# NikolausDemmel/rootba

Hardware: NVIDIA H100
Metric: ms/LM-iter (linearize+QR+PCG) on BAL at 1/2/4/8 H100 vs CPU ref (lower is better)
Workload: dtype f32

## Files before the change

### rootba_b200/csrc/assembled.cuh

```cuda
#pragma once

#include "kernels.cuh"

namespace rba {

template <class S>
__global__ void __launch_bounds__(256) k_rcs_terms(const S* __restrict__ panel, const AsmTerm* __restrict__ terms, long long nt,
                                                   int damping, S* __restrict__ stage, const int* __restrict__ done) {
  using V2 = typename ST<S>::V2;
  if (*done) return;
  const int lane = threadIdx.x & 31;
  const int g = lane / 9, p = lane - 9 * g;
  if (lane >= 27) return;
  const long long warps = (long long)gridDim.x * (blockDim.x >> 5);
  for (long long w = 3 * (blockIdx.x * (long long)(blockDim.x >> 5) + (threadIdx.x >> 5)) + g; w < nt; w += 3 * warps) {
    const AsmTerm at = terms[w];
    const int n = at.meta & 0x7fff, lg = (at.meta >> 15) & 7, KP = at.meta >> 18, G = 1 << lg;
    const int ia = at.ij & 0xffff, ib = at.ij >> 16;
    const int ca = 9 * ia + p, pa = ca >> 1;
    const int off_a = 2 * ((pa >> lg) * 32 + (pa & (G - 1))) + (ca & 1);
    const int cb0 = 9 * ib, pb0 = cb0 >> 1;
    const bool odd = cb0 & 1;
    int off_b[5];
#pragma unroll
// ... 19 lines not shown
    S* o = stage + 81 * (size_t)w + 9 * p;
#pragma unroll
    for (int q = 0; q < 9; ++q) o[q] = acc[q];
  }
}

template <class S>
__global__ void k_rcs_combine(const int* __restrict__ blk_ptr, const int* __restrict__ wpos, int nblk, const S* __restrict__ stage,
                              S* __restrict__ out, const int* __restrict__ done) {
  if (*done) return;
  const long long i = blockIdx.x * (long long)blockDim.x + threadIdx.x;
  if (i >= 81LL * nblk) return;
  const int bi = (int)(i / 81), e = (int)(i - 81LL * bi);
  const S* st = stage + e;
  S s = 0;
  for (int t = blk_ptr[bi]; t < blk_ptr[bi + 1]; ++t) s += st[81 * (size_t)wpos[t]];
  out[i] = s;
}

constexpr int DMP_WARPS = 4;
constexpr int DMP_BATCH = 16;
template <class S>
__global__ void __launch_bounds__(DMP_WARPS * 32) k_rcs_damping(const int* __restrict__ blk_ptr, const int2* __restrict__ terms, int nblk,
                                                                 const S* __restrict__ dmp, const S* __restrict__ base,
                                                                 const int2* __restrict__ pos, S* __restrict__ out,
                                                                 const int* __restrict__ done) {
  constexpr int B = DMP_BATCH, NV = 28 * sizeof(S) / 16;
  constexpr int ROUNDS = (2 * B * NV + 31) / 32;
  __shared__ __align__(16) S rec[DMP_WARPS][B][2][28];
  if (*done) return;
  const int w = threadIdx.x >> 5, lane = threadIdx.x & 31;
  const int bi = blockIdx.x * DMP_WARPS + w;
  if (bi >= nblk) return;
  const bool own = lane < 27;
  const int p = lane / 3, q = 3 * (lane - 3 * p);
  S s[3] = {0, 0, 0};
  if (own) {
#pragma unroll
    for (int u = 0; u < 3; ++u) s[u] = base[81 * (size_t)bi + 3 * lane + u];
  }
  int4* rv = reinterpret_cast<int4*>(&rec[w][0][0][0]);
  const int t1 = blk_ptr[bi + 1];
  for (int t0 = blk_ptr[bi]; t0 < t1; t0 += B) {
    const int nb = min(B, t1 - t0);
    int4 v[ROUNDS];
#pragma unroll
    for (int c = 0; c < ROUNDS; ++c) {
      const int i = lane + 32 * c, r = i / NV, k = i - r * NV;
      v[c] = make_int4(0, 0, 0, 0);
      if (i < 2 * nb * NV) {
        const int2 tt = __ldg(terms + t0 + (r >> 1));
        v[c] = __ldg(reinterpret_cast<const int4*>(dmp + 28 * (size_t)(r & 1 ? tt.y : tt.x)) + k);
      }
    }
#pragma unroll
    for (int c = 0; c < ROUNDS; ++c)
      if (lane + 32 * c < 2 * nb * NV) rv[lane + 32 * c] = v[c];
    __syncwarp();
    if (own) {
      for (int j = 0; j < nb; ++j) {
        const S* a = rec[w][j][0];
        const S* b = rec[w][j][1];
#pragma unroll
        for (int u = 0; u < 3; ++u) {
          S t = fma(a[p], b[q + u], S(0));
          t = fma(a[9 + p], b[9 + q + u], t);
          t = fma(a[18 + p], b[18 + q + u], t);
          s[u] += t;
        }
      }
    }
    __syncwarp();
  }
  if (own) {
    S* o = out + 81 * (size_t)pos[bi].x + 3 * lane;
#pragma unroll
    for (int u = 0; u < 3; ++u) o[u] = s[u];
  }
}

template <class S>
__global__ void k_rcs_mirror(const int2* __restrict__ pos, int nblk, S* val, const int* __restrict__ done) {
  if (*done) return;
  const long long i = blockIdx.x * (long long)blockDim.x + threadIdx.x;
  if (i >= 81LL * nblk) return;
  const int bi = (int)(i / 81), e = (int)(i - 81LL * bi);
  const int2 ps = pos[bi];
  if (ps.y >= 0) val[81 * (size_t)ps.y + e] = val[81 * (size_t)ps.x + 9 * (e % 9) + e / 9];
}

constexpr int SPMV_WARPS = 4;
constexpr int SPMV_UNROLL = 4;
template <class S>
__global__ void __launch_bounds__(SPMV_WARPS * 32) k_rcs_spmv(const int* __restrict__ row_ptr, const int* __restrict__ col,
                                                               const S* __restrict__ val, const S* __restrict__ x, S* __restrict__ y,
                                                               const int* done, int pdl) {
  __shared__ S part[SPMV_WARPS][81];
  if (done && *reinterpret_cast<const volatile int*>(done)) return;
  const int row = blockIdx.x, w = threadIdx.x >> 5, lane = threadIdx.x & 31;
  const int k0 = row_ptr[row], k1 = row_ptr[row + 1];
  int qe[3];
#pragma unroll
  for (int u = 0; u < 3; ++u) qe[u] = (lane + 32 * u) % 9;
  if (pdl) asm volatile("griddepcontrol.wait;" ::: "memory");
  if (done && *done) return;
  if (pdl) asm volatile("griddepcontrol.launch_dependents;" ::: "memory");
  S acc[3] = {0, 0, 0};
  for (int k = k0 + w; k < k1; k += SPMV_WARPS * SPMV_UNROLL) {
    S v[SPMV_UNROLL][3], xv[SPMV_UNROLL][3];
#pragma unroll
    for (int j = 0; j < SPMV_UNROLL; ++j) {
      const int kk = k + SPMV_WARPS * j;
      const bool in = kk < k1;
      const S* blk = val + 81 * (size_t)(in ? kk : k0);
      const S* xc = x + 9 * (size_t)(in ? __ldg(col + kk) : 0);
#pragma unroll
      for (int u = 0; u < 3; ++u) {
        const bool e_in = in && lane + 32 * u < 81;
        v[j][u] = e_in ? __ldg(blk + lane + 32 * u) : S(0);
        xv[j][u] = e_in ? __ldcg(xc + qe[u]) : S(0);
      }
    }
#pragma unroll
    for (int j = 0; j < SPMV_UNROLL; ++j)
#pragma unroll
      for (int u = 0; u < 3; ++u) acc[u] = fma(v[j][u], xv[j][u], acc[u]);
  }
#pragma unroll
  for (int u = 0; u < 3; ++u)
    if (lane + 32 * u < 81) part[w][lane + 32 * u] = acc[u];
  __syncthreads();
  if (threadIdx.x < 9) {
    const int p = threadIdx.x;
    S s = 0;
#pragma unroll
    for (int ww = 0; ww < SPMV_WARPS; ++ww)
#pragma unroll
      for (int q = 0; q < 9; ++q) s += part[ww][9 * p + q];
    y[9 * (size_t)row + p] = s;
  }
}

}
```

### rootba_b200/csrc/solver.cu

```cuda
#include <cuda_runtime.h>
#include <dlfcn.h>

#include <cstdio>
#include <cstdlib>
#include <cstring>
#include <chrono>
#include <array>
#include <limits>
#include <memory>
#include <string>
#include <vector>

#include "../../include/rootba_b200.h"
#include "../host/bal_io_fast.hpp"
#include "kernels.cuh"
#include "covariance.cuh"
#include "assembled.cuh"
#include "groups.cuh"
#include "nccl_dyn.hpp"

namespace rba {

thread_local std::string g_err;

// ... 152 lines not shown
  S* d_pair_ov = nullptr;
  int n_lmp = 0, lmp_cap = 0;
  int* d_lmp_slot = nullptr;
  int* d_lmp_of_lm = nullptr;
  int* d_lmp_lm = nullptr;
  S* d_lmp_mean = nullptr;
  S* d_lmp_L = nullptr;
  S* d_lmp_Lg = nullptr;
  int n_groups = 0;
  std::vector<int> h_grp_lead;
  std::vector<uint8_t> h_fixed;
  int* d_grp_lead = nullptr; int* d_grp_ptr = nullptr; int* d_grp_mem = nullptr;
  uint8_t* d_grp_fixed = nullptr;
  S* d_grp_ve = nullptr;
  S* d_grp_y = nullptr;
  S* d_obs_W = nullptr;
  rba_stage_timings tm{};
  EventPair ev_stage1, ev_stage2, ev_precond, ev_pcg, ev_backsub, ev_update, ev_error, ev_mv, ev_user;
  long long launches = 0;
  long long lin_l0 = 0, solve_l0 = 0, apply_l0 = 0;
  NcclApi* nccl = nullptr;
  ncclComm_t comm = nullptr;
  char* peer_mem = nullptr;
  size_t peer_bytes = 0;
  PeerComm pc{};
  bool peer_ok = false;
  int ar_seq = 0, c_seq = 0, s_seq = 0;
  std::vector<void*> ipc_opened;
  bool cov_ready = false;
  int cov_nblk = 0;
  IntPair* d_cov_blk_cam = nullptr; int* d_cov_blk_ptr = nullptr; IntPair* d_cov_terms = nullptr;
  int* d_cov_lm_slot0 = nullptr; int* d_cov_lm_n = nullptr;
  bool asm_on = false, su_valid = false, s_valid = false, su_new = false;
  int asm_nblk = 0, asm_switch = 0; long long asm_nt = 0, asm_nnzb = 0;
  AsmTerm* d_asm_terms = nullptr; int* d_asm_wpos = nullptr; int* d_asm_blk_ptr = nullptr; IntPair* d_asm_pos = nullptr;
  IntPair* d_asm_slots = nullptr;
  int* d_asm_row_ptr = nullptr; int* d_asm_col = nullptr;
  S* d_asm_stage = nullptr; S* d_asm_Su = nullptr; S* d_asm_S = nullptr;

  ~Solver() override {
    if (comm && nccl) nccl->CommDestroy(comm);
    for (void* p : ipc_opened) cudaIpcCloseMemHandle(p);
    for (void* p : allocs) cudaFree(p);
    if (h_prog) cudaFreeHost(h_prog);
    if (h_state) cudaFreeHost(h_state);
    if (h_res) cudaFreeHost(h_res);
    for (EventPair* e : {&ev_stage1, &ev_stage2, &ev_precond, &ev_pcg, &ev_backsub, &ev_update, &ev_error, &ev_mv, &ev_user}) {
      if (e->a) cudaEventDestroy(e->a);
      if (e->b) cudaEventDestroy(e->b);
    }
    for (auto& e : poll_ev) if (e) cudaEventDestroy(e);
    if (stream) cudaStreamDestroy(stream);
  }

  template <class T>
  int dalloc(T** p, size_t count, bool zero = true) {
    const size_t bytes = std::max<size_t>(count, 1) * sizeof(T);
    void* q = nullptr;
    CU(cudaMalloc(&q, bytes));
    allocs.push_back(q);
    device_bytes += bytes;
    if (zero) CU(cudaMemsetAsync(q, 0, bytes, stream));
    *p = (T*)q;
    return RBA_OK;
  }
  int dfree(void* q) {
    if (!q) return RBA_OK;
    allocs.erase(std::find(allocs.begin(), allocs.end(), q));
    CU(cudaFree(q));
    return RBA_OK;
  }
// ... 38 lines not shown
    TRY(alloc_buffers());
    TRY(setup_assembled());
    TRY(setup_kernels());
    CU(cudaStreamSynchronize(stream));
    return RBA_OK;
  }

  int validate_options(const rba_solver_opts& o) {
    opt = o;
    if (opt.nranks < 1 || opt.rank < 0 || opt.rank >= opt.nranks) { g_err = "bad rank/nranks"; return RBA_ERR_INVALID_ARGUMENT; }
    if (opt.operator_form != 0 && opt.operator_form != 1) { g_err = "operator_form must be 0 (dense) or 1 (implicit)"; return RBA_ERR_INVALID_ARGUMENT; }
    if (opt.solver_type < 0 || opt.solver_type > 2) { g_err = "solver_type must be 0 (SQUARE_ROOT), 1 (SCHUR_COMPLEMENT) or 2 (POWER_SCHUR_COMPLEMENT)"; return RBA_ERR_INVALID_ARGUMENT; }
    if (opt.solver_type == 2 && opt.nranks > 1) { g_err = "POWER_SCHUR_COMPLEMENT runs on one GPU (the power-series vector kernel has no peer exchange yet)"; return RBA_ERR_UNSUPPORTED; }
    if (opt.stage2_form != 0 && opt.stage2_form != 1) { g_err = "stage2_form must be 0 (Q2 panel, reference) or 1 (orthogonality identity)"; return RBA_ERR_INVALID_ARGUMENT; }
    if (opt.pcg_check_period <= 0) opt.pcg_check_period = 4;
    if (opt.residual_reset_period <= 0) opt.residual_reset_period = 10;
    if (opt.power_order <= 0) opt.power_order = 20;
    panels = opt.operator_form == 0 && opt.solver_type == 0;
    ko.use_valid_projections_only = opt.use_valid_projections_only;
    ko.robust_norm = opt.robust_norm;
    ko.write_panel = panels;
    ko.huber = opt.huber_parameter;
    ko.jacobi_eps = opt.jacobi_scaling_epsilon > 0 ? opt.jacobi_scaling_epsilon : (double)ST<S>::eps_sqrt();
    return RBA_OK;
  }
  bool panel_form() const { return panels && opt.stage2_form == 0; }

  void read_test_hooks() {
    if (const char* e = getenv("RBA_PCG_PARTIALS")) pcg_partials = atoi(e) != 0;
    if (const char* e = getenv("RBA_PCG_CLUSTER")) pcg_cluster = std::max(1, std::min(atoi(e), 16));
    if (const char* e = getenv("RBA_PEER_AR")) peer_ar = atoi(e) != 0;
    if (const char* e = getenv("RBA_ASSEMBLED_RCS")) asm_hook = atoi(e) != 0;
    if (const char* e = getenv("RBA_ASSEMBLED_AT")) asm_at = std::max(0, atoi(e));
  }

  int upload_layout(const rba_problem_view* pv) {
    nc = pv->num_cameras;
    nl_total = pv->num_landmarks;
    nobs_total = pv->lm_obs_offset[nl_total];
    std::string msg = build_layout(nc, nl_total, pv->lm_obs_offset, pv->obs_cam_idx, opt.rank, opt.nranks, KPMAX, L);
    if (!msg.empty()) { g_err = msg; return RBA_ERR_INVALID_ARGUMENT; }
    std::vector<S> xy((size_t)2 * L.nslots, S(0));
    const S* src = (const S*)pv->obs_xy;
    for (int s = 0; s < L.nslots; ++s)
      if (L.slot_obs[s] >= 0) { xy[2 * (size_t)s] = src[2 * L.slot_obs[s]]; xy[2 * (size_t)s + 1] = src[2 * L.slot_obs[s] + 1]; }
    TileInfo* d_tiles; int* d_sorted; int* d_slot_cam; int* d_slot_lm; S* d_xy;
    TRY(upload(&d_tiles, L.tiles));
    TRY(upload(&d_sorted, L.sorted_lm));
    TRY(upload(&d_slot_cam, L.slot_cam));
    TRY(upload(&d_slot_lm, L.slot_lm));
    TRY(upload(&d_xy, xy));
    D.tiles = d_tiles; D.ntiles = (int)L.tiles.size(); D.sorted_lm = d_sorted;
    D.slot_cam = d_slot_cam; D.slot_lm = d_slot_lm; D.slot_xy = d_xy; D.nslots = L.nslots; D.nc = nc;
    TRY(upload(&d_csr_obs_slots, L.csr_obs.slots));
    TRY(upload(&d_csr_obs_items, L.csr_obs.items));
    TRY(upload(&d_csr_obs_item_ptr, L.csr_obs.cam_item_ptr));
    n_obs_items = (int)L.csr_obs.items.size();
    if (L.csr_y_is_obs) {
      d_csr_y_slots = d_csr_obs_slots; d_csr_y_items = d_csr_obs_items; d_csr_y_item_ptr = d_csr_obs_item_ptr;
      n_y_items = n_obs_items;
    } else {
      TRY(upload(&d_csr_y_slots, L.csr_y.slots));
      TRY(upload(&d_csr_y_items, L.csr_y.items));
      TRY(upload(&d_csr_y_item_ptr, L.csr_y.cam_item_ptr));
      n_y_items = (int)L.csr_y.items.size();
    }
// ... 762 lines not shown
  }

  int precond_blocks(int mode, S* dst, const S* addend, bool reduce_ranks) {
    const int g = (n_pb_items + 127) / 128;
    switch (mode) {
      case 0: k_precond_partial<S, 0><<<g, 128, 0, stream>>>(D.jp, (const S*)nullptr, d_csr_obs_slots, d_pb_items, n_pb_items, D.pblk); break;
      case 1: k_precond_partial<S, 1><<<g, 128, 0, stream>>>(D.jp, D.q1d, d_csr_obs_slots, d_pb_items, n_pb_items, D.pblk); break;
      case 2: k_precond_partial<S, 2><<<g, 128, 0, stream>>>(D.dmp, (const S*)nullptr, d_csr_obs_slots, d_pb_items, n_pb_items, D.pblk); break;
      default: k_precond_partial<S, 3><<<g, 128, 0, stream>>>(D.blk0, (const S*)nullptr, d_csr_obs_slots, d_pb_items, n_pb_items, D.pblk); break;
    }
    k_precond_final<S><<<(45 * nc + 255) / 256, 256, 0, stream>>>(D.pblk, d_pb_item_ptr, nc, addend, dst);
    launches += 2;
    return reduce_ranks ? allreduce(dst, (size_t)81 * nc) : RBA_OK;
  }

  enum class Handover {
    Assembled,
    Partials,
    Counter,
    Peer,
    Nccl,
  };
  Handover handover() const {
    if (s_valid) return Handover::Assembled;
    if (n_groups) return opt.nranks > 1 ? Handover::Nccl : Handover::Counter;
    if (opt.nranks > 1) return peer_ok ? Handover::Peer : Handover::Nccl;
    const bool vec_cached = 9 * ((nc + pcg_cluster - 1) / pcg_cluster) <= VEC_THREADS * VEC_EPT;
    return pcg_partials && vec_cached && opt.solver_type != 2 ? Handover::Partials : Handover::Counter;
  }
  int apply_operator(const S* xvec, Handover h, bool in_solve, int e0_only = 0) {
    const int* done = in_solve ? &d_state->done : nullptr;
    const bool pdl = in_solve;
    ++tm.matvec_launches;
    if (h == Handover::Assembled)
      return launch_ex(k_rcs_spmv<S>, nc, SPMV_WARPS * 32, 0, pdl, 1, (const int*)d_asm_row_ptr, (const int*)d_asm_col, (const S*)d_asm_S, xvec, D.y, done, (int)pdl);
    if (panels) {
      if (L.n_items_large > 0) {
        k_matvec_large<S, K4_WARPS, KPMAX><<<grid_for(L.n_items_large, K4_WARPS, 4), K4_WARPS * 32, k4_smem_small, stream>>>(
            D, d_items, 0, L.n_items_large, L.k4_scratch_per_warp, xvec, done);
        ++launches;
      }
      const bool p = pdl && L.n_items_large == 0;
      if (n_dealt > L.n_items_large)
        TRY(launch_ex(k_matvec_small_tma<S, K4_WARPS, K4_NS, K4_STAGE>, tma_grid, K4_WARPS * 32, K4_SMEM_TMA, p, 1, D, (const MatvecItem*)d_items, L.n_items_large, n_dealt, xvec, done, (int)p));
    } else {
      const int ntl = (int)L.tiles.size();
      const bool p = pdl && imp_tile_split == ntl;
      if (imp_tile_split > 0)
        TRY(launch_ex((k_matvec_implicit_tma<S, IMP_WARPS, IMP_MAXSLOTS, IMP_NS>), imp_grid, IMP_WARPS * 32, imp_smem, p, 1, D, imp_tile_split, xvec, done, (int)p, e0_only));
      if (imp_tile_split < ntl)
        TRY(launch_ex(k_matvec_implicit<S>, (ntl - imp_tile_split + TILE_WARPS - 1) / TILE_WARPS, TILE_WARPS * 32, 0, false, 1, D, imp_tile_split, xvec, done, 0, e0_only));
    }
    const int grid = grid_for(n_op_items, 8, 8);
    if (h == Handover::Partials)
      return launch_ex(k_cam_reduce<S>, grid, 256, 0, pdl, 1, (const S*)D.yobs, op_slots, op_items, n_op_items, D.partial, done, (int)pdl);
    if (h == Handover::Peer) ++ar_seq;
    if (h == Handover::Nccl) CU(cudaMemsetAsync(D.y, 0, (size_t)9 * nc * sizeof(S), stream));
    auto kern = h == Handover::Peer ? k_cam_reduce_final<S, true> : k_cam_reduce_final<S, false>;
    TRY(launch_ex(kern, grid, 256, 0, pdl, 1, (const S*)D.yobs, op_slots, op_items, n_op_items, op_item_ptr, D.partial, d_cam_cnt, D.y, done, (int)pdl, pc, ar_seq, nc));
    return h == Handover::Nccl ? allreduce(D.y, (size_t)9 * nc) : RBA_OK;
  }
  int matvec_launch(const S* xvec, bool clear_y) {
    const Handover h = handover() == Handover::Assembled ? Handover::Assembled : Handover::Counter;
    if (clear_y && h == Handover::Counter) CU(cudaMemsetAsync(D.y, 0, (size_t)9 * nc * sizeof(S), stream));
    return apply_operator(xvec, h, false);
  }
  int pcg_vec(int i, int mode, bool pdl, int is_last, S lambda, bool fused_ar = false, bool from_partials = false) {
    PeerComm c = pc;
// ... 113 lines not shown
    Handover h = handover();
    if (h == Handover::Counter) CU(cudaMemsetAsync(D.y, 0, (size_t)9 * nc * sizeof(S), stream));
    if (power) return power_enqueue(h, inc_out);
    rc = start(ev_pcg); if (rc) return rc;
    CU(cudaMemsetAsync(d_state, 0, sizeof(PcgState), stream));
    const int max_it = std::max(opt.max_linear_solver_iterations, 1);
    const int period = opt.residual_reset_period;
    const int depth = opt.pcg_check_period;
    h_prog[0] = 0; h_prog[1] = 0;
    ar_seq = (++pcg_solve_id) * (2 * max_it + 4);
    rc = pcg_vec(0, 3, false, 0, lambda); if (rc) return rc;
    auto enqueue_iteration = [&](int i) -> int {
      const int is_last = (i == max_it) ? 1 : 0;
      if (i % period == 0) {
        TRY(pcg_step(i, 1, 0, lambda, h));
        return pcg_step(i, 2, is_last, lambda, h);
      }
      return pcg_step(i, 0, is_last, lambda, h);
    };
    if (h == Handover::Nccl) {
      TRY(enqueue_polled(max_it, depth, enqueue_iteration));
    } else {
      volatile int* prog = h_prog;
      for (int i = 1; i <= max_it; ++i) {
        unsigned spins = 0;
        while (!prog[1] && i - prog[0] > depth) {
          if ((++spins & 0xffffu) == 0 && cudaStreamQuery(stream) != cudaErrorNotReady) break;
        }
        if (prog[1] && i - prog[0] > depth) break;
        if (asm_on && i == asm_switch) {
          su_new = !su_valid;
          if (su_new) assemble(0);
          assemble(1);
          su_valid = s_valid = true;
          h = handover();
        }
        rc = enqueue_iteration(i); if (rc) return rc;
      }
    }
    if (n_groups) TRY(group_expand(D.inc, D.inc, false));
    CU(cudaMemcpyAsync(&h_state[0], d_state, sizeof(PcgState), cudaMemcpyDeviceToHost, stream));
    if (inc_out) CU(cudaMemcpyAsync(inc_out, D.inc, (size_t)9 * nc * sizeof(S), cudaMemcpyDeviceToHost, stream));
    rc = stop(ev_pcg); if (rc) return rc;
    have_inc = true;
    new_linearization_point = false;
    return RBA_OK;
  }
  int solve_finish(rba_cg_summary* cg) {
    CU(cudaGetLastError());
    tm.stage2_time = elapsed(ev_stage2);
    tm.compute_preconditioner_time = elapsed(ev_precond);
    tm.solve_reduced_system_time = elapsed(ev_pcg);
    tm.kernel_launches = launches - solve_l0;
    if (cg) {
      cg->termination_type = h_state[0].term;
      cg->num_iterations = h_state[0].iter;
      cg->reason = h_state[0].reason;
      cg->num_matvecs = h_state[0].iter + h_state[0].iter / opt.residual_reset_period;
    }
    if (s_valid && h_state[0].iter < asm_switch) {
      s_valid = false;
      if (su_new) su_valid = false;
    }
    if (h_state[0].reason == 99) {
      g_err = "PCG: a peer rank did not publish its operator output in time (peer-memory exchange timed out)";
      return RBA_ERR_NCCL;
    }
// ... 213 lines not shown
    CU(cudaGetLastError());
    return RBA_OK;
  }

  int time_matvec(int reps, double* sec) override {
    if (!linearized || !damping_valid) { g_err = "rba_time_matvec needs rba_linearize + rba_solve first"; return RBA_ERR_STATE; }
    TRY(matvec_launch(D.p, false));
    TRY(start(ev_mv));
    for (int r = 0; r < reps; ++r) TRY(matvec_launch(D.p, false));
    TRY(stop(ev_mv));
    CU(cudaStreamSynchronize(stream));
    CU(cudaGetLastError());
    *sec = elapsed(ev_mv) / std::max(reps, 1);
    tm.matvec_time = *sec;
    return RBA_OK;
  }

  int timer_start() override { return start(ev_user); }
  int timer_stop(double* sec) override {
    int rc = stop(ev_user); if (rc) return rc;
    CU(cudaStreamSynchronize(stream));
    *sec = elapsed(ev_user);
    return RBA_OK;
  }
  void* stream_ptr() override { return (void*)stream; }
  int synchronize() override { CU(cudaStreamSynchronize(stream)); return RBA_OK; }

  bool asm_candidate() const { return asm_hook && opt.nranks == 1 && panels; }
  int setup_assembled() {
    if (!asm_candidate()) return RBA_OK;
    PairList P;
    const std::string msg = build_pair_list(L, P);
    if (!msg.empty()) { g_err = msg; return RBA_ERR_UNSUPPORTED; }
    AsmPlan A;
    plan_assembled(L, P, sizeof(S), A);
    if (!A.fits) return RBA_OK;
    size_t free_b = 0, total_b = 0;
    CU(cudaMemGetInfo(&free_b, &total_b));
    if ((size_t)A.device_bytes + ((size_t)256 << 20) > free_b) return RBA_OK;
    TRY(upload(&d_asm_terms, A.terms));
    TRY(upload(&d_asm_wpos, P.wpos));
    TRY(upload(&d_asm_slots, P.terms));
    TRY(upload(&d_asm_blk_ptr, P.blk_ptr));
    TRY(upload(&d_asm_pos, A.pos));
    TRY(upload(&d_asm_row_ptr, A.row_ptr));
    TRY(upload(&d_asm_col, A.col));
    TRY(dalloc(&d_asm_stage, (size_t)A.nt * 81, false));
    TRY(dalloc(&d_asm_Su, (size_t)A.nblk * 81));
    TRY(dalloc(&d_asm_S, (size_t)A.nnzb * 81));
    asm_nt = A.nt; asm_nblk = (int)A.nblk; asm_nnzb = A.nnzb;
    asm_switch = asm_at > 0 ? asm_at : A.switch_iteration;
    asm_on = true;
    return RBA_OK;
  }
  void assemble(int damping) {
    const int* done = &d_state->done;
    const unsigned per_entry = (unsigned)((81LL * asm_nblk + 255) / 256);
    if (damping) {
      k_rcs_damping<S><<<(asm_nblk + DMP_WARPS - 1) / DMP_WARPS, DMP_WARPS * 32, 0, stream>>>(
          d_asm_blk_ptr, (const int2*)d_asm_slots, asm_nblk, D.dmp, d_asm_Su, (const int2*)d_asm_pos, d_asm_S, done);
      k_rcs_mirror<S><<<per_entry, 256, 0, stream>>>((const int2*)d_asm_pos, asm_nblk, d_asm_S, done);
    } else {
      const int grid = (int)std::max<long long>(1, std::min<long long>((asm_nt + 23) / 24, (long long)sm_count * 16));
      k_rcs_terms<S><<<grid, 256, 0, stream>>>(D.panel, d_asm_terms, asm_nt, 0, d_asm_stage, done);
      k_rcs_combine<S><<<per_entry, 256, 0, stream>>>(d_asm_blk_ptr, d_asm_wpos, asm_nblk, d_asm_stage, d_asm_Su, done);
    }
    launches += 2;
  }

  template <class T>
  int cov_upload(T** p, const std::vector<T>& v) {
    void* q = nullptr;
    CU(cudaMalloc(&q, std::max<size_t>(v.size(), 1) * sizeof(T)));
    allocs.push_back(q);
    if (!v.empty()) CU(cudaMemcpy(q, v.data(), v.size() * sizeof(T), cudaMemcpyHostToDevice));
    *p = (T*)q;
    return RBA_OK;
  }
  int cov_build_lists() {
    if (cov_ready) return RBA_OK;
    PairList P;
    const std::string msg = build_pair_list(L, P);
    if (!msg.empty()) { g_err = msg; return RBA_ERR_UNSUPPORTED; }
    TRY(cov_upload(&d_cov_blk_cam, P.blk_cam));
    TRY(cov_upload(&d_cov_blk_ptr, P.blk_ptr));
    TRY(cov_upload(&d_cov_terms, P.terms));
    TRY(cov_upload(&d_cov_lm_slot0, P.slot0));
    TRY(cov_upload(&d_cov_lm_n, P.nn));
    cov_nblk = (int)P.blk_cam.size();
    cov_ready = true;
    return RBA_OK;
  }
  template <bool TA, bool TB>
  void cov_gemm(long long M, long long N, long long K, double alpha, const double* A, long long lda, const double* B, long long ldb,
// ... 505 lines not shown
```

### rootba_b200/csrc/kernels.cuh

```cuda
#pragma once

#include <cooperative_groups.h>
#include <cuda_runtime.h>

#include <cfloat>
#include <cmath>
#include <cstdint>

#include "layout.hpp"

namespace rba {

template <class S> struct ST;
template <> struct ST<float> {
  using V2 = float2;
  using V4 = float4;
  __host__ __device__ static float eps_sqrt() { return 0.0031622776601683794f; }
  __host__ __device__ static float eps() { return 1e-5f; }
  __host__ __device__ static float tiny() { return FLT_MIN; }
};
template <> struct ST<double> {
  using V2 = double2;
  using V4 = double4;
  __host__ __device__ static double eps_sqrt() { return 1e-5; }
// ... 1572 lines not shown
      const V2 v = __ldg(prow + (size_t)(r * KP + k) * 32);
      const int c = 2 * lane + 64 * k;
      d += v.x * xs[c] + v.y * xs[c + 1];
    }
    d = warp_sum(d);
    for (int k = 0; k < KP; ++k) {
      const V2 v = __ldg(prow + (size_t)(r * KP + k) * 32);
      const int c = 2 * lane + 64 * k;
      ys[c] += d * v.x;
      ys[c + 1] += d * v.y;
    }
  }
  __syncwarp();
  for (int c = lane; c < ncols; c += 32) D.yobs[9 * (size_t)it.yslot_base + c] = ys[c];
  __syncwarp();
}

__device__ __forceinline__ uint32_t smem_u32(const void* p) { return (uint32_t)__cvta_generic_to_shared(p); }
__device__ __forceinline__ void mbar_init(uint64_t* bar, uint32_t count) {
  asm volatile("mbarrier.init.shared::cta.b64 [%0], %1;" ::"r"(smem_u32(bar)), "r"(count) : "memory");
}
__device__ __forceinline__ void mbar_fence_init() {
  asm volatile("fence.mbarrier_init.release.cluster;" ::: "memory");
  asm volatile("fence.proxy.async.shared::cta;" ::: "memory");
}
__device__ __forceinline__ void mbar_expect_tx(uint64_t* bar, uint32_t bytes) {
  asm volatile("mbarrier.arrive.expect_tx.shared::cta.b64 _, [%0], %1;" ::"r"(smem_u32(bar)), "r"(bytes) : "memory");
}
__device__ __forceinline__ uint64_t l2_evict_first_policy() {
  uint64_t pol;
  asm volatile("createpolicy.fractional.L2::evict_first.b64 %0, 1.0;" : "=l"(pol));
  return pol;
}
__device__ __forceinline__ void bulk_g2s(void* dst, const void* src, uint32_t bytes, uint64_t* bar, uint64_t policy) {
  asm volatile("cp.async.bulk.shared::cluster.global.mbarrier::complete_tx::bytes.L2::cache_hint [%0], [%1], %2, [%3], %4;" ::"r"(
                   smem_u32(dst)),
               "l"(src), "r"(bytes), "r"(smem_u32(bar)), "l"(policy)
               : "memory");
}
__device__ __forceinline__ void mbar_wait(uint64_t* bar, uint32_t parity) {
  uint32_t ok;
  const uint32_t a = smem_u32(bar);
  do {
    asm volatile("{\n .reg .pred p;\n mbarrier.try_wait.parity.shared::cta.b64 p, [%1], %2;\n selp.u32 %0, 1, 0, p;\n}"
                 : "=r"(ok)
                 : "r"(a), "r"(parity)
                 : "memory");
  } while (!ok);
}

template <class S>
struct PanelStream {
  const S* src;
  int rows_left;
  int row_scalars;
  int rows_per_stage;
  int next_item;
  unsigned issued;
  uint64_t policy;
};

template <class S, int NS, int STAGE_BYTES>
__device__ __forceinline__ bool stream_produce(PanelStream<S>& ps, const DevPtrs<S>& D, const MatvecItem* __restrict__ items,
                                               int item_end, int item_stride, unsigned char* ring, uint64_t* bars, int lane) {
  if (ps.rows_left == 0) {
    if (ps.next_item >= item_end) return false;
// ... 1291 lines not shown
```

### rootba_b200/csrc/layout.hpp

```cpp
#pragma once

#include <algorithm>
#include <cmath>
#include <cstdint>
#include <limits>
#include <numeric>
#include <string>
#include <utility>
#include <vector>

namespace rba {

struct TileInfo {
  long long panel_off;
  int slot_base;
  int lm_base;
  short n;
  short G;
  short KP;
  short nvalid;
};

struct MatvecItem {
  int tile;
// ... 294 lines not shown
  pass(tmp, idx, true);
  tmp.clear(); tmp.shrink_to_fit();
  P.terms.resize(raw.size());
  for (size_t t = 0; t < idx.size(); ++t) P.terms[t] = raw[idx[t]];
  P.wpos.swap(idx);
  for (size_t t = 0; t < P.terms.size(); ++t) {
    const IntPair cc{L.slot_cam[P.terms[t].x], L.slot_cam[P.terms[t].y]};
    if (t == 0 || cc.x != P.blk_cam.back().x || cc.y != P.blk_cam.back().y) {
      P.blk_cam.push_back(cc);
      P.blk_ptr.push_back((int)t);
    }
  }
  P.blk_ptr.push_back((int)P.terms.size());
  return "";
}

struct AsmTerm {
  long long base;
  int ij, meta;
};
inline AsmTerm pack_asm_term(long long base, int ia, int ib, int n, int G, int KP) {
  int lg = 0;
  while ((1 << lg) < G) ++lg;
  return {base, ia | ib << 16, n | lg << 15 | KP << 18};
}

constexpr long long ASM_STAGE_BYTES = (long long)2 << 30;

inline int asm_switch_iteration(long long nt, long long panel_scalars, long long s_bytes, int scalar_size) {
  const double staged = 4.0 * (double)nt * 81 * scalar_size, saved = (double)panel_scalars * scalar_size - (double)s_bytes;
  return 1 + (int)std::ceil(2.0 * staged / std::max(saved, 1.0));
}

struct AsmPlan {
  long long nt = 0, nblk = 0, nnzb = 0, s_bytes = 0, device_bytes = 0;
  bool fits = false;
  int switch_iteration = 0;
  std::vector<int> row_ptr;
  std::vector<int> col;
  std::vector<IntPair> pos;
  std::vector<AsmTerm> terms;
};

inline void plan_assembled(const Layout& L, const PairList& P, int scalar_size, AsmPlan& A) {
  A = AsmPlan();
  const int nc = L.nc;
  A.nblk = (long long)P.blk_cam.size();
  A.nt = (long long)P.terms.size();
  long long ndiag = 0;
  for (const IntPair& c : P.blk_cam) ndiag += c.x == c.y;
  A.nnzb = 2 * A.nblk - ndiag;
  A.s_bytes = A.nnzb * 81 * scalar_size;
  A.switch_iteration = asm_switch_iteration(A.nt, L.panel_scalars, A.s_bytes, scalar_size);
  A.fits = 4 * A.s_bytes <= L.panel_scalars * scalar_size && 81 * A.nt * scalar_size <= ASM_STAGE_BYTES;
  if (!A.fits) return;
  A.device_bytes = A.s_bytes + (A.nblk + A.nt) * 81 * scalar_size + A.nt * (long long)(sizeof(AsmTerm) + sizeof(int) + sizeof(IntPair)) +
                   (A.nblk + A.nnzb + nc + 2) * (long long)sizeof(int) + A.nblk * (long long)sizeof(IntPair);
  A.row_ptr.assign((size_t)nc + 1, 0);
  A.col.resize((size_t)A.nnzb);
  for (const IntPair& c : P.blk_cam) { ++A.row_ptr[c.x + 1]; if (c.x != c.y) ++A.row_ptr[c.y + 1]; }
  for (int c = 0; c < nc; ++c) A.row_ptr[c + 1] += A.row_ptr[c];
  std::vector<int> fill(A.row_ptr.begin(), A.row_ptr.end() - 1);
  A.pos.resize((size_t)A.nblk);
  for (long long b = 0; b < A.nblk; ++b) {
    const IntPair c = P.blk_cam[b];
    const int lo = fill[c.x]++;
    A.col[lo] = c.y;
    int up = -1;
    if (c.x != c.y) { up = fill[c.y]++; A.col[up] = c.x; }
    A.pos[b] = {lo, up};
  }
  A.terms.reserve((size_t)A.nt);
  for (int lm = 0; lm < L.nl_local; ++lm) {
    const int sidx = L.sorted_of_lm[lm];
    const TileInfo& T = L.tiles[L.tile_of_sorted[sidx]];
    const int g = sidx - T.lm_base;
    for (int a = 0; a < T.n; ++a)
      for (int b = 0; b <= a; ++b) A.terms.push_back(pack_asm_term(T.panel_off + 2LL * g * T.G, a, b, T.n, T.G, T.KP));
  }
}

}
```

Baseline: 6.013.

## Fuse mirror into damping kernel and add dedicated diagonal-block damping kernel

The separate mirror kernel is removed. The off-diagonal damping kernel now writes both the lower block and its transpose into the upper position directly. Diagonal blocks, which can carry many terms, are handled by a new block-per-diagonal kernel that prefetches term records into shared memory one batch ahead and uses the symmetric a^T a product. This removes a launch and a read-back pass and spreads the long diagonal sums across 81 threads instead of 27 lanes. The cost is strided transposed stores and an extra kernel with a software-pipelined loop.

New measurement: 5.982 (median of 6 runs). No clear change (-0.5%).

```diff
diff --git a/rootba_b200/csrc/assembled.cuh b/rootba_b200/csrc/assembled.cuh
--- a/rootba_b200/csrc/assembled.cuh
+++ b/rootba_b200/csrc/assembled.cuh
@@ -75,6 +75,8 @@
   const int w = threadIdx.x >> 5, lane = threadIdx.x & 31;
   const int bi = blockIdx.x * DMP_WARPS + w;
   if (bi >= nblk) return;
+  const int2 ps = __ldg(pos + bi);
+  if (ps.y < 0) return;
   const bool own = lane < 27;
   const int p = lane / 3, q = 3 * (lane - 3 * p);
   S s[3] = {0, 0, 0};
@@ -116,20 +118,65 @@
     __syncwarp();
   }
   if (own) {
-    S* o = out + 81 * (size_t)pos[bi].x + 3 * lane;
-#pragma unroll
-    for (int u = 0; u < 3; ++u) o[u] = s[u];
-  }
-}
-
-template <class S>
-__global__ void k_rcs_mirror(const int2* __restrict__ pos, int nblk, S* val, const int* __restrict__ done) {
-  if (*done) return;
-  const long long i = blockIdx.x * (long long)blockDim.x + threadIdx.x;
-  if (i >= 81LL * nblk) return;
-  const int bi = (int)(i / 81), e = (int)(i - 81LL * bi);
-  const int2 ps = pos[bi];
-  if (ps.y >= 0) val[81 * (size_t)ps.y + e] = val[81 * (size_t)ps.x + 9 * (e % 9) + e / 9];
+    S* lo = out + 81 * (size_t)ps.x + 3 * lane;
+    S* up = out + 81 * (size_t)ps.y + p;
+#pragma unroll
+    for (int u = 0; u < 3; ++u) {
+      lo[u] = s[u];
+      up[9 * (q + u)] = s[u];
+    }
+  }
+}
+
+constexpr int DIAG_THREADS = 96;
+constexpr int DIAG_BATCH = 32;
+template <class S>
+__global__ void __launch_bounds__(DIAG_THREADS) k_rcs_damping_diag(const int* __restrict__ diag, const int* __restrict__ blk_ptr,
+                                                                    const int2* __restrict__ terms, const S* __restrict__ dmp,
+                                                                    const S* __restrict__ base, const int2* __restrict__ pos,
+                                                                    S* __restrict__ out, const int* __restrict__ done) {
+  constexpr int B = DIAG_BATCH, NV = 28 * sizeof(S) / 16;
+  constexpr int ROUNDS = (B * NV + DIAG_THREADS - 1) / DIAG_THREADS;
+  __shared__ __align__(16) S rec[B][28];
+  if (*done) return;
+  const int bi = __ldg(diag + blockIdx.x), e = threadIdx.x;
+  const bool own = e < 81;
+  const int p = e / 9, q = e - 9 * p;
+  S s = own ? base[81 * (size_t)bi + e] : S(0);
+  const int t0 = __ldg(blk_ptr + bi), t1 = __ldg(blk_ptr + bi + 1);
+  int4 v[ROUNDS];
+  int4* rv = reinterpret_cast<int4*>(&rec[0][0]);
+  for (int t = t0 - B; t < t1; t += B) {
+    if (t >= t0) {
+      __syncthreads();
+#pragma unroll
+      for (int c = 0; c < ROUNDS; ++c)
+        if (e + DIAG_THREADS * c < min(B, t1 - t) * NV) rv[e + DIAG_THREADS * c] = v[c];
+      __syncthreads();
+    }
+    const int nf = min(B, t1 - t - B);
+#pragma unroll
+    for (int c = 0; c < ROUNDS; ++c) {
+      const int i = e + DIAG_THREADS * c, r = i / NV, k = i - r * NV;
+      v[c] = make_int4(0, 0, 0, 0);
+      if (i < nf * NV) {
+        const int slot = __ldg(reinterpret_cast<const int*>(terms + t + B + r));
+        v[c] = __ldg(reinterpret_cast<const int4*>(dmp + 28 * (size_t)slot) + k);
+      }
+    }
+    if (t < t0) continue;
+    const int nb = min(B, t1 - t);
+    if (own) {
+      for (int j = 0; j < nb; ++j) {
+        const S* a = rec[j];
+        S u = fma(a[p], a[q], S(0));
+        u = fma(a[9 + p], a[9 + q], u);
+        u = fma(a[18 + p], a[18 + q], u);
+        s += u;
+      }
+    }
+  }
+  if (own) out[81 * (size_t)__ldg(&pos[bi].x) + e] = s;
 }
 
 constexpr int SPMV_WARPS = 4;
diff --git a/rootba_b200/csrc/solver.cu b/rootba_b200/csrc/solver.cu
--- a/rootba_b200/csrc/solver.cu
+++ b/rootba_b200/csrc/solver.cu
@@ -208,10 +208,10 @@
   IntPair* d_cov_blk_cam = nullptr; int* d_cov_blk_ptr = nullptr; IntPair* d_cov_terms = nullptr;
   int* d_cov_lm_slot0 = nullptr; int* d_cov_lm_n = nullptr;
   bool asm_on = false, su_valid = false, s_valid = false, su_new = false;
-  int asm_nblk = 0, asm_switch = 0; long long asm_nt = 0, asm_nnzb = 0;
+  int asm_nblk = 0, asm_switch = 0, asm_ndiag = 0; long long asm_nt = 0, asm_nnzb = 0;
   AsmTerm* d_asm_terms = nullptr; int* d_asm_wpos = nullptr; int* d_asm_blk_ptr = nullptr; IntPair* d_asm_pos = nullptr;
   IntPair* d_asm_slots = nullptr;
-  int* d_asm_row_ptr = nullptr; int* d_asm_col = nullptr;
+  int* d_asm_row_ptr = nullptr; int* d_asm_col = nullptr; int* d_asm_diag = nullptr;
   S* d_asm_stage = nullptr; S* d_asm_Su = nullptr; S* d_asm_S = nullptr;
 
   ~Solver() override {
@@ -1619,10 +1619,14 @@
     TRY(upload(&d_asm_pos, A.pos));
     TRY(upload(&d_asm_row_ptr, A.row_ptr));
     TRY(upload(&d_asm_col, A.col));
+    std::vector<int> diag;
+    for (long long b = 0; b < A.nblk; ++b)
+      if (A.pos[b].y < 0) diag.push_back((int)b);
+    TRY(upload(&d_asm_diag, diag));
     TRY(dalloc(&d_asm_stage, (size_t)A.nt * 81, false));
     TRY(dalloc(&d_asm_Su, (size_t)A.nblk * 81));
     TRY(dalloc(&d_asm_S, (size_t)A.nnzb * 81));
-    asm_nt = A.nt; asm_nblk = (int)A.nblk; asm_nnzb = A.nnzb;
+    asm_nt = A.nt; asm_nblk = (int)A.nblk; asm_nnzb = A.nnzb; asm_ndiag = (int)diag.size();
     asm_switch = asm_at > 0 ? asm_at : A.switch_iteration;
     asm_on = true;
     return RBA_OK;
@@ -1633,7 +1637,8 @@
     if (damping) {
       k_rcs_damping<S><<<(asm_nblk + DMP_WARPS - 1) / DMP_WARPS, DMP_WARPS * 32, 0, stream>>>(
           d_asm_blk_ptr, (const int2*)d_asm_slots, asm_nblk, D.dmp, d_asm_Su, (const int2*)d_asm_pos, d_asm_S, done);
-      k_rcs_mirror<S><<<per_entry, 256, 0, stream>>>((const int2*)d_asm_pos, asm_nblk, d_asm_S, done);
+      k_rcs_damping_diag<S><<<asm_ndiag, DIAG_THREADS, 0, stream>>>(d_asm_diag, d_asm_blk_ptr, (const int2*)d_asm_slots, D.dmp, d_asm_Su,
+                                                                   (const int2*)d_asm_pos, d_asm_S, done);
     } else {
       const int grid = (int)std::max<long long>(1, std::min<long long>((asm_nt + 23) / 24, (long long)sm_count * 16));
       k_rcs_terms<S><<<grid, 256, 0, stream>>>(D.panel, d_asm_terms, asm_nt, 0, d_asm_stage, done);
```

## Rewrite assembled SpMV as persistent load-balanced kernel with bulk-copy pipeline

Applied to the files above, without the earlier changes.

Replaces the one-CTA-per-row block SpMV with a persistent grid sized by occupancy. Rows are dealt to CTAs with LPT balancing and split into fixed-size chunks. Matrix blocks are streamed into shared memory via cp.async.bulk with a three-stage mbarrier pipeline and an L2 evict-last hint, and x entries are gathered into a shared window. The aim is to cut load imbalance across rows, launch-wide tail effects and global-load latency in PCG matvecs. In exchange it adds many block-wide syncs per chunk, host-side planning, and disables PDL on the first launch after reassembly.

New measurement: 5.952 before, 5.565 after, median of 6. 1.07x faster.

```diff
diff --git a/rootba_b200/csrc/assembled.cuh b/rootba_b200/csrc/assembled.cuh
--- a/rootba_b200/csrc/assembled.cuh
+++ b/rootba_b200/csrc/assembled.cuh
@@ -132,56 +132,138 @@
   if (ps.y >= 0) val[81 * (size_t)ps.y + e] = val[81 * (size_t)ps.x + 9 * (e % 9) + e / 9];
 }
 
-constexpr int SPMV_WARPS = 4;
-constexpr int SPMV_UNROLL = 4;
-template <class S>
-__global__ void __launch_bounds__(SPMV_WARPS * 32) k_rcs_spmv(const int* __restrict__ row_ptr, const int* __restrict__ col,
-                                                               const S* __restrict__ val, const S* __restrict__ x, S* __restrict__ y,
-                                                               const int* done, int pdl) {
-  __shared__ S part[SPMV_WARPS][81];
-  if (done && *reinterpret_cast<const volatile int*>(done)) return;
-  const int row = blockIdx.x, w = threadIdx.x >> 5, lane = threadIdx.x & 31;
-  const int k0 = row_ptr[row], k1 = row_ptr[row + 1];
+constexpr int SPMV_NS = 3;
+template <class S>
+__global__ void __launch_bounds__(SPMV_CLASSES * 32) k_rcs_spmv(const SpmvChunk* __restrict__ chunks, const int* __restrict__ chunk_ptr,
+                                                                 const int* __restrict__ col, const S* __restrict__ val,
+                                                                 const S* __restrict__ x, S* __restrict__ y, const int* done, int pdl) {
+  constexpr int CH = SPMV_STAGE_BYTES / (81 * (int)sizeof(S)), U = CH / SPMV_CLASSES;
+  constexpr int VB = CH * 81 * (int)sizeof(S) + 16;
+  constexpr int XWIN = sizeof(S) == 4 ? 256 : 128;
+  static_assert(CH % SPMV_CLASSES == 0 && VB % 16 == 0 && XWIN >= CH, "k_rcs_spmv stage layout");
+  __shared__ __align__(128) unsigned char sval[SPMV_NS][VB];
+  __shared__ S sx[XWIN * 9];
+  __shared__ int scol[XWIN];
+  __shared__ __align__(8) uint64_t bars[SPMV_NS];
+  __shared__ S part[SPMV_CLASSES][81];
+  __shared__ int quit;
+  if (threadIdx.x == 0) {
+    quit = done && *reinterpret_cast<const volatile int*>(done);
+    if (!quit) {
+      for (int s = 0; s < SPMV_NS; ++s) mbar_init(&bars[s], 1);
+      mbar_fence_init();
+    }
+  }
+  __syncthreads();
+  if (quit) return;
+  const int c0 = chunk_ptr[blockIdx.x], n = chunk_ptr[blockIdx.x + 1] - c0;
+  const int w = threadIdx.x >> 5, lane = threadIdx.x & 31;
+  const uint64_t policy = l2_evict_last_policy();
+  constexpr uintptr_t A16 = ~(uintptr_t)15;
+  auto request = [&](int i) {
+    const SpmvChunk ch = chunks[c0 + i];
+    const int s = i % SPMV_NS;
+    const uintptr_t v0 = (uintptr_t)(val + 81 * (size_t)ch.kb) & A16, v1 = ((uintptr_t)(val + 81 * (size_t)ch.ke) + 15) & A16;
+    mbar_expect_tx(&bars[s], (uint32_t)(v1 - v0));
+    if (v1 > v0) bulk_g2s(sval[s], (const void*)v0, (uint32_t)(v1 - v0), &bars[s], policy);
+  };
+  auto window = [&](int i0, int& nblk) {
+    int i = i0, off = 0;
+    for (; i < n; ++i) {
+      const SpmvChunk ch = chunks[c0 + i];
+      const int nb = ch.ke - ch.kb;
+      if (off + nb > XWIN) break;
+      if ((i - i0) % SPMV_CLASSES == w)
+        for (int t = lane; t < nb; t += 32) scol[off + t] = __ldg(col + ch.kb + t);
+      off += nb;
+    }
+    nblk = off;
+    return i;
+  };
+  auto gather_x = [&](int nblk) {
+    constexpr int B = 8;
+    for (int t0 = threadIdx.x; t0 < 9 * nblk; t0 += B * SPMV_CLASSES * 32) {
+      S v[B];
+#pragma unroll
+      for (int j = 0; j < B; ++j) {
+        const int t = t0 + j * SPMV_CLASSES * 32;
+        v[j] = t < 9 * nblk ? __ldcg(x + 9 * (size_t)scol[t / 9] + t % 9) : S(0);
+      }
+#pragma unroll
+      for (int j = 0; j < B; ++j) {
+        const int t = t0 + j * SPMV_CLASSES * 32;
+        if (t < 9 * nblk) sx[t] = v[j];
+      }
+    }
+  };
+  const int primed = min(n, SPMV_NS);
+  if (threadIdx.x == 0)
+    for (int i = 0; i < primed; ++i) request(i);
+  int nblk = 0;
+  int wend = window(0, nblk);
+  if (pdl) asm volatile("griddepcontrol.wait;" ::: "memory");
+  if (done && *done) {
+    for (int i = 0; i < primed; ++i) mbar_wait(&bars[i], 0);
+    return;
+  }
+  if (pdl) asm volatile("griddepcontrol.launch_dependents;" ::: "memory");
+  __syncthreads();
+  gather_x(nblk);
+  __syncthreads();
   int qe[3];
 #pragma unroll
   for (int u = 0; u < 3; ++u) qe[u] = (lane + 32 * u) % 9;
-  if (pdl) asm volatile("griddepcontrol.wait;" ::: "memory");
-  if (done && *done) return;
-  if (pdl) asm volatile("griddepcontrol.launch_dependents;" ::: "memory");
   S acc[3] = {0, 0, 0};
-  for (int k = k0 + w; k < k1; k += SPMV_WARPS * SPMV_UNROLL) {
-    S v[SPMV_UNROLL][3], xv[SPMV_UNROLL][3];
-#pragma unroll
-    for (int j = 0; j < SPMV_UNROLL; ++j) {
-      const int kk = k + SPMV_WARPS * j;
-      const bool in = kk < k1;
-      const S* blk = val + 81 * (size_t)(in ? kk : k0);
-      const S* xc = x + 9 * (size_t)(in ? __ldg(col + kk) : 0);
+  for (int i = 0, jb = 0; i < n; ++i) {
+    if (i == wend) {
+      wend = window(i, nblk);
+      __syncthreads();
+      gather_x(nblk);
+      __syncthreads();
+      jb = 0;
+    }
+    const SpmvChunk ch = chunks[c0 + i];
+    const int s = i % SPMV_NS, nb = ch.ke - ch.kb;
+    if (ch.flags & SPMV_FIRST) acc[0] = acc[1] = acc[2] = 0;
+    mbar_wait(&bars[s], (i / SPMV_NS) & 1u);
+    const S* vs = reinterpret_cast<const S*>(sval[s] + ((uintptr_t)(val + 81 * (size_t)ch.kb) & 15));
+    const S* xs = sx + 9 * jb;
+    S v[U][3], xv[U][3];
+#pragma unroll
+    for (int j = 0; j < U; ++j) {
+      const int b = w + SPMV_CLASSES * j;
 #pragma unroll
       for (int u = 0; u < 3; ++u) {
-        const bool e_in = in && lane + 32 * u < 81;
-        v[j][u] = e_in ? __ldg(blk + lane + 32 * u) : S(0);
-        xv[j][u] = e_in ? __ldcg(xc + qe[u]) : S(0);
-      }
-    }
-#pragma unroll
-    for (int j = 0; j < SPMV_UNROLL; ++j)
-#pragma unroll
-      for (int u = 0; u < 3; ++u) acc[u] = fma(v[j][u], xv[j][u], acc[u]);
-  }
-#pragma unroll
-  for (int u = 0; u < 3; ++u)
-    if (lane + 32 * u < 81) part[w][lane + 32 * u] = acc[u];
-  __syncthreads();
-  if (threadIdx.x < 9) {
-    const int p = threadIdx.x;
-    S s = 0;
-#pragma unroll
-    for (int ww = 0; ww < SPMV_WARPS; ++ww)
-#pragma unroll
-      for (int q = 0; q < 9; ++q) s += part[ww][9 * p + q];
-    y[9 * (size_t)row + p] = s;
-  }
-}
-
-}
+        const bool e_in = b < nb && lane + 32 * u < 81;
+        v[j][u] = e_in ? vs[81 * b + lane + 32 * u] : S(0);
+        xv[j][u] = e_in ? xs[9 * b + qe[u]] : S(0);
+      }
+    }
+#pragma unroll
+    for (int j = 0; j < U; ++j)
+      if (w + SPMV_CLASSES * j < nb) {
+#pragma unroll
+        for (int u = 0; u < 3; ++u) acc[u] = fma(v[j][u], xv[j][u], acc[u]);
+      }
+    jb += nb;
+    if (ch.flags & SPMV_LAST) {
+#pragma unroll
+      for (int u = 0; u < 3; ++u)
+        if (lane + 32 * u < 81) part[w][lane + 32 * u] = acc[u];
+      __syncthreads();
+      if (threadIdx.x < 9) {
+        const int p = threadIdx.x;
+        S t = 0;
+#pragma unroll
+        for (int c = 0; c < SPMV_CLASSES; ++c)
+#pragma unroll
+          for (int q = 0; q < 9; ++q) t += part[c][9 * p + q];
+        y[9 * (size_t)ch.row + p] = t;
+      }
+    }
+    __syncthreads();
+    if (threadIdx.x == 0 && i + SPMV_NS < n) request(i + SPMV_NS);
+  }
+}
+
+}
diff --git a/rootba_b200/csrc/kernels.cuh b/rootba_b200/csrc/kernels.cuh
--- a/rootba_b200/csrc/kernels.cuh
+++ b/rootba_b200/csrc/kernels.cuh
@@ -1628,6 +1628,11 @@
   asm volatile("createpolicy.fractional.L2::evict_first.b64 %0, 1.0;" : "=l"(pol));
   return pol;
 }
+__device__ __forceinline__ uint64_t l2_evict_last_policy() {
+  uint64_t pol;
+  asm volatile("createpolicy.fractional.L2::evict_last.b64 %0, 1.0;" : "=l"(pol));
+  return pol;
+}
 __device__ __forceinline__ void bulk_g2s(void* dst, const void* src, uint32_t bytes, uint64_t* bar, uint64_t policy) {
   asm volatile("cp.async.bulk.shared::cluster.global.mbarrier::complete_tx::bytes.L2::cache_hint [%0], [%1], %2, [%3], %4;" ::"r"(
                    smem_u32(dst)),
diff --git a/rootba_b200/csrc/layout.hpp b/rootba_b200/csrc/layout.hpp
--- a/rootba_b200/csrc/layout.hpp
+++ b/rootba_b200/csrc/layout.hpp
@@ -350,6 +350,44 @@
   return 1 + (int)std::ceil(2.0 * staged / std::max(saved, 1.0));
 }
 
+constexpr int SPMV_CLASSES = 4;
+constexpr int SPMV_STAGE_BYTES = 32 * 81 * 4;
+constexpr int spmv_chunk_blocks(int scalar_size) { return SPMV_STAGE_BYTES / (81 * scalar_size); }
+struct SpmvChunk {
+  int row, kb, ke;
+  int flags;
+};
+constexpr int SPMV_FIRST = 1, SPMV_LAST = 2;
+struct SpmvDeal {
+  int ctas = 0;
+  std::vector<int> chunk_ptr;
+  std::vector<SpmvChunk> chunks;
+};
+inline void deal_spmv(const std::vector<int>& row_ptr, int ctas, int chunk_blocks, SpmvDeal& D) {
+  D = SpmvDeal();
+  const int nrows = (int)row_ptr.size() - 1;
+  D.ctas = std::max(1, std::min(ctas, nrows));
+  std::vector<long long> cost((size_t)std::max(nrows, 0));
+  for (int r = 0; r < nrows; ++r) cost[r] = row_ptr[r + 1] - row_ptr[r];
+  const std::vector<int> order = deal_lpt(cost, D.ctas);
+  D.chunk_ptr.assign((size_t)D.ctas + 1, 0);
+  for (int b = 0; b < D.ctas; ++b) {
+    D.chunk_ptr[b] = (int)D.chunks.size();
+    for (size_t k = b; k < order.size(); k += D.ctas) {
+      const int r = order[k];
+      if (r < 0) break;
+      const int k0 = row_ptr[r], k1 = row_ptr[r + 1];
+      int kb = k0;
+      do {
+        const int ke = std::min(k1, kb + chunk_blocks);
+        D.chunks.push_back({r, kb, ke, (kb == k0 ? SPMV_FIRST : 0) | (ke == k1 ? SPMV_LAST : 0)});
+        kb = ke;
+      } while (kb < k1);
+    }
+  }
+  D.chunk_ptr[D.ctas] = (int)D.chunks.size();
+}
+
 struct AsmPlan {
   long long nt = 0, nblk = 0, nnzb = 0, s_bytes = 0, device_bytes = 0;
   bool fits = false;
@@ -358,9 +396,10 @@
   std::vector<int> col;
   std::vector<IntPair> pos;
   std::vector<AsmTerm> terms;
-};
-
-inline void plan_assembled(const Layout& L, const PairList& P, int scalar_size, AsmPlan& A) {
+  SpmvDeal spmv;
+};
+
+inline void plan_assembled(const Layout& L, const PairList& P, int scalar_size, AsmPlan& A, int spmv_ctas = 0) {
   A = AsmPlan();
   const int nc = L.nc;
   A.nblk = (long long)P.blk_cam.size();
@@ -372,8 +411,8 @@
   A.switch_iteration = asm_switch_iteration(A.nt, L.panel_scalars, A.s_bytes, scalar_size);
   A.fits = 4 * A.s_bytes <= L.panel_scalars * scalar_size && 81 * A.nt * scalar_size <= ASM_STAGE_BYTES;
   if (!A.fits) return;
-  A.device_bytes = A.s_bytes + (A.nblk + A.nt) * 81 * scalar_size + A.nt * (long long)(sizeof(AsmTerm) + sizeof(int) + sizeof(IntPair)) +
-                   (A.nblk + A.nnzb + nc + 2) * (long long)sizeof(int) + A.nblk * (long long)sizeof(IntPair);
+  A.device_bytes = A.s_bytes + 16 + (A.nblk + A.nt) * 81 * scalar_size + A.nt * (long long)(sizeof(AsmTerm) + sizeof(int) + sizeof(IntPair)) +
+                   (A.nblk + 1 + A.nnzb) * (long long)sizeof(int) + A.nblk * (long long)sizeof(IntPair);
   A.row_ptr.assign((size_t)nc + 1, 0);
   A.col.resize((size_t)A.nnzb);
   for (const IntPair& c : P.blk_cam) { ++A.row_ptr[c.x + 1]; if (c.x != c.y) ++A.row_ptr[c.y + 1]; }
@@ -396,6 +435,10 @@
     for (int a = 0; a < T.n; ++a)
       for (int b = 0; b <= a; ++b) A.terms.push_back(pack_asm_term(T.panel_off + 2LL * g * T.G, a, b, T.n, T.G, T.KP));
   }
-}
-
-}
+  if (spmv_ctas > 0) {
+    deal_spmv(A.row_ptr, spmv_ctas, spmv_chunk_blocks(scalar_size), A.spmv);
+    A.device_bytes += (long long)A.spmv.chunks.size() * (long long)sizeof(SpmvChunk) + (A.spmv.ctas + 1) * (long long)sizeof(int);
+  }
+}
+
+}
diff --git a/rootba_b200/csrc/solver.cu b/rootba_b200/csrc/solver.cu
--- a/rootba_b200/csrc/solver.cu
+++ b/rootba_b200/csrc/solver.cu
@@ -211,8 +211,10 @@
   int asm_nblk = 0, asm_switch = 0; long long asm_nt = 0, asm_nnzb = 0;
   AsmTerm* d_asm_terms = nullptr; int* d_asm_wpos = nullptr; int* d_asm_blk_ptr = nullptr; IntPair* d_asm_pos = nullptr;
   IntPair* d_asm_slots = nullptr;
-  int* d_asm_row_ptr = nullptr; int* d_asm_col = nullptr;
+  int* d_asm_col = nullptr;
   S* d_asm_stage = nullptr; S* d_asm_Su = nullptr; S* d_asm_S = nullptr;
+  SpmvChunk* d_spmv_chunks = nullptr; int* d_spmv_chunk_ptr = nullptr; int spmv_grid = 0, spmv_cap = 0;
+  bool s_fresh = false;
 
   ~Solver() override {
     if (comm && nccl) nccl->CommDestroy(comm);
@@ -317,6 +319,7 @@
     if (const char* e = getenv("RBA_PEER_AR")) peer_ar = atoi(e) != 0;
     if (const char* e = getenv("RBA_ASSEMBLED_RCS")) asm_hook = atoi(e) != 0;
     if (const char* e = getenv("RBA_ASSEMBLED_AT")) asm_at = std::max(0, atoi(e));
+    if (const char* e = getenv("RBA_SPMV_CTAS")) spmv_cap = std::max(1, atoi(e));
   }
 
   int upload_layout(const rba_problem_view* pv) {
@@ -1145,8 +1148,12 @@
     const int* done = in_solve ? &d_state->done : nullptr;
     const bool pdl = in_solve;
     ++tm.matvec_launches;
-    if (h == Handover::Assembled)
-      return launch_ex(k_rcs_spmv<S>, nc, SPMV_WARPS * 32, 0, pdl, 1, (const int*)d_asm_row_ptr, (const int*)d_asm_col, (const S*)d_asm_S, xvec, D.y, done, (int)pdl);
+    if (h == Handover::Assembled) {
+      const bool p = pdl && !s_fresh;
+      s_fresh = false;
+      return launch_ex(k_rcs_spmv<S>, spmv_grid, SPMV_CLASSES * 32, 0, p, 1, (const SpmvChunk*)d_spmv_chunks, (const int*)d_spmv_chunk_ptr,
+                       (const int*)d_asm_col, (const S*)d_asm_S, xvec, D.y, done, (int)p);
+    }
     if (panels) {
       if (L.n_items_large > 0) {
         k_matvec_large<S, K4_WARPS, KPMAX><<<grid_for(L.n_items_large, K4_WARPS, 4), K4_WARPS * 32, k4_smem_small, stream>>>(
@@ -1326,7 +1333,7 @@
           su_new = !su_valid;
           if (su_new) assemble(0);
           assemble(1);
-          su_valid = s_valid = true;
+          su_valid = s_valid = s_fresh = true;
           h = handover();
         }
         rc = enqueue_iteration(i); if (rc) return rc;
@@ -1606,8 +1613,11 @@
     PairList P;
     const std::string msg = build_pair_list(L, P);
     if (!msg.empty()) { g_err = msg; return RBA_ERR_UNSUPPORTED; }
+    int occ = 0;
+    CU(cudaOccupancyMaxActiveBlocksPerMultiprocessor(&occ, k_rcs_spmv<S>, SPMV_CLASSES * 32, 0));
     AsmPlan A;
-    plan_assembled(L, P, sizeof(S), A);
+    const int ctas = std::max(1, occ) * sm_count;
+    plan_assembled(L, P, sizeof(S), A, spmv_cap > 0 ? std::min(spmv_cap, ctas) : ctas);
     if (!A.fits) return RBA_OK;
     size_t free_b = 0, total_b = 0;
     CU(cudaMemGetInfo(&free_b, &total_b));
@@ -1617,11 +1627,13 @@
     TRY(upload(&d_asm_slots, P.terms));
     TRY(upload(&d_asm_blk_ptr, P.blk_ptr));
     TRY(upload(&d_asm_pos, A.pos));
-    TRY(upload(&d_asm_row_ptr, A.row_ptr));
     TRY(upload(&d_asm_col, A.col));
+    TRY(upload(&d_spmv_chunks, A.spmv.chunks));
+    TRY(upload(&d_spmv_chunk_ptr, A.spmv.chunk_ptr));
+    spmv_grid = A.spmv.ctas;
     TRY(dalloc(&d_asm_stage, (size_t)A.nt * 81, false));
     TRY(dalloc(&d_asm_Su, (size_t)A.nblk * 81));
-    TRY(dalloc(&d_asm_S, (size_t)A.nnzb * 81));
+    TRY(dalloc(&d_asm_S, (size_t)A.nnzb * 81 + 16 / sizeof(S)));
     asm_nt = A.nt; asm_nblk = (int)A.nblk; asm_nnzb = A.nnzb;
     asm_switch = asm_at > 0 ? asm_at : A.switch_iteration;
     asm_on = true;
```
